# r4dl/StopThePop-Rasterization

Measured on AMD Instinct MI355X. Metric: fwd+bwd frames/sec at 1920×1080, 1M Gaussians; PSNR vs reference, higher is better.
Workload: dtype f32

## Files before the change

### stopthepop-rasterization_amd/csrc/stp_api.hip

```cpp
#include "stp_internal.h"

#include <algorithm>
#include <atomic>
#include <chrono>
#include <cstdio>
#include <cstdlib>
#include <cstring>
#include <mutex>
#include <string>
#include <unordered_map>
#include <vector>

namespace stp {

static thread_local std::string g_last_error;
static bool g_timing = false;

struct StageTimer {
    static constexpr int SETS = 64, EV = 8;
    static constexpr int HIST = 1024;
    struct Set { hipEvent_t ev[EV]; bool have[EV]; bool used; long seq; std::chrono::steady_clock::time_point host[EV]; };
    Set sets[SETS] = {};
    bool created = false;
    int cur = 0;
// ... 603 lines not shown
                const float* cam_pos, float tan_fovx, float tan_fovy, int prefiltered, float* out_color, int* radii, int debug,
                void* stream)
{
    hipStream_t st = (hipStream_t)stream;
    const ForwardSplit split = t_forward_split;
    t_forward_split = ForwardSplit{};
    struct SplitGuard {
        const ForwardSplit& s; hipStream_t st; bool done = false;
        ~SplitGuard() { if (s.armed && !done) (void)hipEventRecord(s.event, st); }
    } split_guard{split, st};
    if (!settings || !geometry_alloc || !binning_alloc || !image_alloc) return fail(STP_ERR_INVALID_ARGUMENT, "null settings or allocator");
    if (P < 0 || width <= 0 || height <= 0) return fail(STP_ERR_INVALID_ARGUMENT, "bad sizes");
    if (P == 0) return 0;
    if (!means3D || !opacities || !background || !viewmatrix || !projmatrix || !inv_viewprojmatrix || !cam_pos || !out_color)
        return fail(STP_ERR_INVALID_ARGUMENT, "null required input");
    if (int rc = check_settings(*settings, false)) return rc;
    if (!colors_precomp && !shs) return fail(STP_ERR_INVALID_ARGUMENT, "neither SHs nor precomputed colours given");
    if (!cov3D_precomp && !(scales && rotations)) return fail(STP_ERR_INVALID_ARGUMENT, "neither scale/rotation nor precomputed covariance given");
    const bool with_inv = requires_depth_along_ray(*settings);
    if (with_inv && !(scales && rotations)) return fail(STP_ERR_NEEDS_SCALE_ROTATION, "sorted modes need scales and rotations");

    FrameParams f;
    fill_frame(f, P, D, M, background, width, height, *settings, means3D, shs, colors_precomp, opacities, scales, scale_modifier,
               rotations, cov3D_precomp, viewmatrix, projmatrix, inv_viewprojmatrix, cam_pos, tan_fovx, tan_fovy, prefiltered);

    size_t geom_bytes = 0;
    carve_geometry(nullptr, (size_t)P, with_inv, &geom_bytes);
    char* geom_ptr = (char*)geometry_alloc(geometry_user, geom_bytes);
    if (!geom_ptr) return fail(STP_ERR_ALLOC, "geometry allocator returned NULL");
    GeometryState g = carve_geometry(geom_ptr, (size_t)P, with_inv, nullptr);
    if (!radii) radii = g.internal_radii;

    Mailbox mb;
    if (int rc = acquire_mailbox(&mb)) return rc;
    const uint64_t gkey = guess_key(f);
    const unsigned gidx = (unsigned)((gkey >> 1) % GUESS_SLOTS);
    SizeGuess& gslot = g_guess[mb.device][gidx];
    uint32_t* const log_need_word = g_mailboxes[mb.device].log_need + gidx;
    size_t img_bytes = 0;
    const bool with_log = uses_blend_log(*settings);
    const int log_depth = with_log ? log_depth_for(gslot, gkey) : 0;
    f.log_depth = log_depth;
    f.log_need = with_log ? log_need_word : nullptr;
    const uint32_t log_tag = (uint32_t)((gkey >> 40) & 0xFFFFu) | 1u;
    f.log_tag = log_tag;
    carve_image(nullptr, width, height, f.ty0, f.ty1, log_depth, &img_bytes);
    char* img_ptr = (char*)image_alloc(image_user, img_bytes);
    if (!img_ptr) return fail(STP_ERR_ALLOC, "image allocator returned NULL");
    ImageState img = carve_image(img_ptr, width, height, f.ty0, f.ty1, log_depth, nullptr);

    static const char* const sort_env = std::getenv("STP_SORT");
    static const bool tile_local_sort = !(sort_env && std::strcmp(sort_env, "radix") == 0);
    static const bool atomic_bin = sort_env && std::strcmp(sort_env, "counters") == 0;

    static const char* const scan_env = std::getenv("STP_SCAN");
    static const bool two_level_scan = !(scan_env && std::strcmp(scan_env, "rocprim") == 0);
    if (!two_level_scan) { g.block_sums = nullptr; g.block_prefix = nullptr; }

    g_timer.begin_forward();
    g_timer.mark(0, st);
    STP_TRY(launch_frame_init(g, img, f.gx * f.ty0, f.gx * (f.ty1 - f.ty0), with_log, atomic_bin, st), "frame init launch");
    STP_TRY(launch_preprocess(f, g, radii, atomic_bin ? img.tile_counts : nullptr, st), "preprocess launch");
    STP_DEBUG_SYNC("preprocess");
    if (!two_level_scan) STP_TRY(launch_scan(f, g, st), "inclusive scan");
    STP_DEBUG_SYNC("scan");
    if (atomic_bin) STP_TRY(launch_tile_scan(f, img, st), "tile scan");

    if (two_level_scan) STP_TRY(launch_block_prefix_mailbox(f, g, mb.dev, mb.ticket, log_need_word, st), "workgroup prefixes + mailbox launch");
    else STP_TRY(launch_mailbox(g.point_offsets + (P - 1), g.status + 1, mb.dev, mb.ticket, log_need_word, st), "mailbox launch");
    STP_TRY(hipEventRecord(mb.ev, st), "record mailbox event");
    SideStream* const side = side_stream(mb.device);
    SideJoin colours{mb.done, st, false};
    static const char* const late_env = std::getenv("STP_COLOUR_LATE");
    static const bool colour_late = !(late_env && late_env[0] == '0');
    auto colour_on_side = [&]() -> int {
        STP_TRY(hipStreamWaitEvent(side->stream, mb.ev, 0), "side stream wait");
        STP_TRY(launch_sh_color(f, g, radii, side->stream), "SH colour launch");
        if (hipError_t e = hipEventRecord(mb.done, side->stream); e != hipSuccess) {
            (void)hipStreamSynchronize(side->stream);
            return fail_hip(e, "record colour event");
        }
        colours.pending = true;
        return 0;
    };
    if (side) {
        if (!colour_late) { if (int rc = colour_on_side()) return rc; }
    } else STP_TRY(launch_sh_color(f, g, radii, st), "SH colour launch");
    static const char* const bin_env = std::getenv("STP_BINNING");
    static const bool speculative = !(bin_env && std::strcmp(bin_env, "exact") == 0);
    const int run_ahead_mode = g_run_ahead.load(std::memory_order_relaxed);
    const bool run_ahead = run_ahead_mode != 0;
    size_t bin_have = 0;
    char* bin_ptr = nullptr;
    const uint32_t guess = (speculative && gslot.key.load(std::memory_order_acquire) == gkey) ? gslot.R.load(std::memory_order_relaxed) : 0u;
    const bool ahead = run_ahead && guess > 0 && (run_ahead_mode == 1 || guess < RUN_AHEAD_AUTO_MAX) && two_level_scan && !atomic_bin && !debug;
    const uint32_t cap = guess + guess / 8 + (ahead ? 1024u : 0u);
    if (guess > 0) {
        carve_binning(nullptr, (size_t)cap, &bin_have);
        bin_ptr = (char*)binning_alloc(binning_user, bin_have);
        if (!bin_ptr) return fail(STP_ERR_ALLOC, "binning allocator returned NULL");
    }
    static const char* const mbx_env = std::getenv("STP_MAILBOX");
    static const bool mbx_spin = !(mbx_env && std::strcmp(mbx_env, "event") == 0);
    auto wait_mailbox = [&]() -> int {
        if (mbx_spin) {
            for (unsigned it = 1;; it++) {
// ... 216 lines not shown
```

### stopthepop-rasterization_amd/csrc/stp_blend.h

```cpp
#pragma once

#include "stp_device.h"

namespace stp {

struct RenderArgs {
    int W, H, gx, ty0, ty1;
    const uint2* ranges;
    const uint32_t* point_list;
    const float2* means2D;
    const float4* conic_opacity;
    const float4* cov3D_inv;
    const float* features;
    const float4* entA;
    const float4* entB;
    const float4* entC;
    const float4* entD;
    const float4* entF;
    const float* inv_vp;
    const float* cam;
    const float* bg;
    float* final_T;
    uint32_t* n_contrib;
    float* out_color;
    const float* pixel_colors;
    const float* dL_dpix;
    float* grad_rec;
    int grad_stride;
    uint32_t* blend_log;
    int log_depth;
    uint32_t* log_need;
    uint32_t log_tag;
    uint32_t* tile_flags;
    const uint32_t* tile_order;
    int flag_mode;
    int debug_depth;
    const float* means3D;
};

typedef uint16_t log_t;
constexpr int LOG_MAX_LIST = 65535;
#ifndef STP_LOG_DEPTH
#define STP_LOG_DEPTH 192
#endif
constexpr int BLEND_LOG_DEPTH = STP_LOG_DEPTH, BLEND_LOG_DEPTH_MIN = 32, BLEND_LOG_DEPTH_MAX = 512;
constexpr int LOG_BLOCK = 4;
constexpr int LOG_PIECE_SHIFT = 3;
constexpr int BLEND_LOG_SPARE = 8;
__host__ __device__ __forceinline__ size_t log_wave_bytes(int depth) { return (size_t)(depth + BLEND_LOG_SPARE) * 64 * sizeof(uint16_t); }
__device__ __forceinline__ char* log_wave_slice(uint32_t* blend_log, int tile, int wave, int depth)
{
    return reinterpret_cast<char*>(blend_log) + (size_t)(tile * 4 + wave) * log_wave_bytes(depth);
}
inline bool log_blocked(const StpSettings& s) { return s.sort_mode == 2; }
template <bool BLOCKED> __device__ __forceinline__ uint32_t log_record_offset(uint32_t j2, uint32_t lane16)
{
    if constexpr (BLOCKED) return (((j2 << 6) & ~(128u * LOG_BLOCK - 1u)) | lane16) | (j2 & (2u * LOG_BLOCK - 2u));
    else return (j2 << 6) | (lane16 >> (LOG_PIECE_SHIFT - 1));
}
struct BlockedLogCursor {
    char* wave;
    uint32_t cap2;
    uint32_t piece;
    uint32_t j2 = 0u;
    uint32_t lo = 0u, hi = 0u;
    __device__ __forceinline__ void append(bool upd, int pay)
    {
        if (upd) {
            lo = __builtin_amdgcn_alignbit(hi, lo, 16);
            hi = __builtin_amdgcn_alignbit((uint32_t)pay, hi, 16);
            if ((j2 & 6u) == 6u && j2 < cap2) *reinterpret_cast<uint2*>(wave + log_record_offset<true>(j2 & ~6u, piece)) = make_uint2(lo, hi);
        }
        j2 += upd ? 2u : 0u;
    }
    __device__ __forceinline__ int records() const { return (int)(j2 >> 1); }
    __device__ __forceinline__ void flush()
    {
        const uint32_t have = (j2 >> 1) & 3u;
        if (have != 0u && (j2 & ~6u) < cap2) {
            const unsigned long long acc = ((((unsigned long long)hi) << 32) | lo) >> (16u * (4u - have));
            *reinterpret_cast<uint2*>(wave + log_record_offset<true>(j2 & ~6u, piece)) = make_uint2((uint32_t)acc, (uint32_t)(acc >> 32));
        }
    }
};

__device__ __forceinline__ void report_log_need(uint32_t* word, int nrec, uint32_t tag)
{
    int m = nrec;
#pragma unroll
    for (int off = 32; off > 0; off >>= 1) m = max(m, __shfl_xor(m, off));
// ... 230 lines not shown
```

### stopthepop-rasterization_amd/csrc/stp_internal.h

```cpp
#pragma once

#include <hip/hip_runtime.h>
#include <cstdint>
#include <cstddef>
#include <cstdlib>
#include <string>

#include "../../include/stp_raster.h"

namespace stp {

constexpr int TILE = 16;
constexpr size_t ALIGN = 256;

enum SortMode { MODE_GLOBAL = 0, MODE_FULL = 1, MODE_KBUFFER = 2, MODE_HIER = 3 };
enum SortOrder { ORDER_Z = 0, ORDER_DISTANCE = 1, ORDER_PTD_CENTER = 2, ORDER_PTD_MAX = 3 };

inline bool uses_blend_log(const StpSettings& s)
{
    return s.record_blend_log != 0 && s.debug_visualization == 0 && (s.sort_mode == MODE_HIER || s.sort_mode == MODE_KBUFFER);
}

inline int subtile_mask_kind(const StpSettings& s)
{
// ... 61 lines not shown
    int log_depth;
};

struct BinningState {
    uint32_t* header;
    uint32_t* point_list;
    uint32_t* point_list_unsorted;
    uint64_t* keys;
    uint64_t* keys_unsorted;
    char* sort_temp;
    size_t sort_temp_bytes;
    float4* entA;
    float4* entB;
    float4* entC;
    float4* entD;
    float4* entF;
};

constexpr uint32_t STP_HEADER_MAGIC_BINNING = 0x42505453u, STP_HEADER_MAGIC_IMAGE = 0x49505453u;
struct NamedOffset { const char* name; size_t offset; size_t count; };

GeometryState carve_geometry(char* base, size_t P, bool with_inv, size_t* total, NamedOffset* names = nullptr, int* n_names = nullptr);
ImageState carve_image(char* base, int W, int H, int ty0, int ty1, int log_depth , size_t* total, NamedOffset* names = nullptr, int* n_names = nullptr);
BinningState carve_binning(char* base, size_t R, size_t* total, NamedOffset* names = nullptr, int* n_names = nullptr);

int blend_log_rows(int depth);
int blend_log_default_depth();
int blend_log_clamp_depth(int d);
size_t scan_temp_bytes(size_t P);
size_t sort_temp_bytes(size_t R);

struct FrameParams {
    int P, D, M, W, H, gx, gy;
    int ty0, ty1;
    float focal_x, focal_y, tan_fovx, tan_fovy, scale_modifier;
    StpSettings s;
    const float* background;
    const float* means3D;
    const float* shs;
    const float* colors_precomp;
    const float* opacities;
    const float* scales;
    const float* rotations;
    const float* cov3D_precomp;
    const float* viewmatrix;
    const float* projmatrix;
    const float* inv_viewprojmatrix;
    const float* cam_pos;
    int prefiltered;
    int log_depth;
    uint32_t* log_need;
    uint32_t log_tag;
    int split_launch = 0;
    int wild_cov;
};

struct BackwardParams {
    const float* pixel_colors;
    const float* dL_dpix;
    float* grad_rec;
    int grad_stride;
    int clear_rec;
    int chunk, chunks;
    float* dL_dmean2D;
    float* dL_dopacity;
    float* dL_dcolor;
    float* dL_dmean3D;
    float* dL_dcov3D;
    float* dL_dsh;
    float* dL_dscale;
    float* dL_drot;
};

hipError_t launch_preprocess(const FrameParams& f, const GeometryState& g, int* radii, uint32_t* tile_counts, hipStream_t st);
hipError_t launch_frame_init(const GeometryState& g, const ImageState& img, int tile0, int n_tiles, bool with_log, bool tile_counters, hipStream_t st);
hipError_t launch_scan(const FrameParams& f, const GeometryState& g, hipStream_t st);
bool tile_order_enabled();
inline bool tile_order_used(const FrameParams& f) { return tile_order_enabled() && f.gx * (f.ty1 - f.ty0) > 1024; }
bool gather_order_enabled();
int gather_order_mode();
hipError_t launch_tile_order(const FrameParams& f, const ImageState& img, hipStream_t st);
hipError_t launch_sh_color(const FrameParams& f, const GeometryState& g, const int* radii, hipStream_t st);
hipError_t launch_mailbox(const uint32_t* last_offset, const uint32_t* status, uint32_t* mailbox_dev, uint32_t ticket, uint32_t* log_need, hipStream_t st);
hipError_t launch_block_prefix_mailbox(const FrameParams& f, const GeometryState& g, uint32_t* mailbox_dev, uint32_t ticket, uint32_t* log_need, hipStream_t st);
hipError_t launch_duplicate(const FrameParams& f, const GeometryState& g, const int* radii, const BinningState& b, uint32_t* tile_cursor, uint32_t cap, uint32_t header_cap, uint32_t* zero_ptr, size_t zero_words, hipStream_t st);
hipError_t launch_tile_scan(const FrameParams& f, const ImageState& img, hipStream_t st);
hipError_t launch_bin_pad(const BinningState& b, const ImageState& img, int R, hipStream_t st);
hipError_t launch_sort(const FrameParams& f, const BinningState& b, int R, bool tile_bits_only, bool zeroed, hipStream_t st);
void sort_zero_region(const BinningState& b, size_t R, uint32_t tiles, uint32_t** ptr, size_t* words);
hipError_t launch_tile_sort_gather(const FrameParams& f, const GeometryState& g, const BinningState& b, const ImageState& img, int R, bool unordered, hipStream_t st);
hipError_t launch_ranges(const FrameParams& f, const BinningState& b, const ImageState& img, int R, hipStream_t st);
hipError_t launch_gather_entries(const FrameParams& f, const GeometryState& g, const BinningState& b, int R, hipStream_t st);
hipError_t launch_render_forward(const FrameParams& f, const GeometryState& g, const BinningState& b, const ImageState& img,
                                 float* out_color, hipStream_t st, std::string* err);
hipError_t launch_render_debug_finish(const FrameParams& f, const ImageState& img, float* out_color, hipStream_t st);
hipError_t launch_render_backward(const FrameParams& f, const GeometryState& g, const BinningState& b, const ImageState& img,
                                  const BackwardParams& bw, hipStream_t st, std::string* err);
hipError_t launch_preprocess_backward(const FrameParams& f, const GeometryState& g, const int* radii, const BackwardParams& bw, hipStream_t st);
hipError_t launch_mark_visible(int P, const float* means3D, const float* viewmatrix, uint8_t* present, hipStream_t st);

uint32_t higher_msb(uint32_t n);

}
```

### stopthepop-rasterization_amd/csrc/stp_render_hier.inc

```
#include "stp_internal.h"
#include "stp_blend.h"

namespace stp {

#ifdef STP_HIER_STATS
static __device__ unsigned long long g_hier_stats[16];
#if defined(STP_INST_MODE) && STP_INST_MODE == 2 && STP_INST_MID == 8
extern "C" int stp_debug_hier_stats(unsigned long long* out16)
{
    hipError_t e = hipMemcpyFromSymbol(out16, HIP_SYMBOL(g_hier_stats), sizeof(unsigned long long) * 16);
    unsigned long long z[16] = {};
    (void)hipMemcpyToSymbol(HIP_SYMBOL(g_hier_stats), z, sizeof(z));
    return (int)e;
}
#endif
#endif

namespace {

#ifndef STP_BWD_WIN
#define STP_BWD_WIN 256
#endif
#ifndef STP_BWD_RING
#define STP_BWD_RING 512
// ... 36 lines not shown
    static __host__ __device__ constexpr size_t wave_mask(int MID) { return ring_cs(MID) + (size_t)BWD_RING * 4; }
    static __host__ __device__ constexpr size_t total(int MID, int mode) { return mode == 1 ? wave_mask(MID) + 16 : hfifo(MID) + 64 * (size_t)HF_CAP * 4; }
};

__device__ __forceinline__ int hier_remap_tile(int wg, int n_wg)
{
    const int q = n_wg >> 3, r = n_wg & 7;
    const int xcd = wg & 7, k = wg >> 3;
    return (xcd < r ? xcd * (q + 1) : r * (q + 1) + (xcd - r) * q) + k;
}

constexpr int MODE_FWD = 0, MODE_BWD = 1, MODE_FWD_RECORD = 2, MODE_FWD_DEPTH = 3;

template <int HEAD, int MID, bool CULL, int MODE, bool FRCP>
__global__ void __launch_bounds__(256, MODE == MODE_BWD ? STP_BWD_WAVES : (HEAD == 4 && MID == 8 && FRCP) ? STP_FWD_WAVES : 4) render_hier_kernel(const RenderArgs a)
{
    constexpr bool FRESH_QUAD = MODE != MODE_BWD && HEAD == 4 && MID == 8 && FRCP && STP_FWD_WAVES >= 5 && CULL;
    constexpr bool BACKWARD = MODE == MODE_BWD;
    constexpr bool RECORD = MODE == MODE_FWD_RECORD;
    constexpr bool DEPTHVIZ = MODE == MODE_FWD_DEPTH;
    constexpr bool USE_POS = true;
    extern __shared__ __attribute__((aligned(16))) char smem[];
    constexpr int OLDN = (MID - 4) / 4;

    const int lane = (int)(threadIdx.x & 63);
    const int w = __builtin_amdgcn_readfirstlane((int)(threadIdx.x >> 6));
    const int s = lane >> 4;
    const int x = lane & 15;
    const int m = x >> 2;
    const int q = x & 3;

    const int rows = a.ty1 - a.ty0;
    const int t = a.tile_order ? (int)a.tile_order[blockIdx.x] : hier_remap_tile((int)blockIdx.x, a.gx * rows);
    const int tile_x = t % a.gx, tile_y = a.ty0 + t / a.gx;
    const uint2 range = a.ranges[tile_y * a.gx + tile_x];
    if constexpr (BACKWARD) {
        if (a.flag_mode == 1 && a.tile_flags[tile_y * a.gx + tile_x] == 0u) return;
    }

    const int cx = tile_x * TILE + 4 * s, cy = tile_y * TILE + 4 * w;
    const int px = cx + 2 * (m & 1) + (q & 1), py = cy + 2 * (m >> 1) + (q >> 1);
    const bool inside = px < a.W && py < a.H;
    bool active = inside;
    if constexpr (!BACKWARD) {
        if (range.y <= range.x) {
            if (inside) {
                const size_t N = (size_t)a.W * a.H, pid = (size_t)a.W * py + px;
                a.final_T[pid] = 1.0f;
                if constexpr (RECORD) a.n_contrib[pid] = 0u;
                if constexpr (DEPTHVIZ) { a.out_color[pid] = 0.0f; a.out_color[N + pid] = 1.0f; }
                else { a.out_color[pid] = a.bg[0]; a.out_color[N + pid] = a.bg[1]; a.out_color[2 * N + pid] = a.bg[2]; }
            }
            return;
        }
    }

    const int st = w * 4 + s;
    auto fresh_lane = [&]() __attribute__((always_inline)) -> int {
        int l;
        asm volatile("v_mbcnt_lo_u32_b32 %0, -1, 0\n\tv_mbcnt_hi_u32_b32 %0, -1, %0" : "=v"(l));
        return l;
    };
#define STP_ROW_VIEW(L)                                                                                                  \
    const int lrow_ = (L);                                               \
    const int x = lrow_ & 15;                                                                                            \
    const int st_r = w * 4 + (lrow_ >> 4);                                                                               \
    float* const tk = reinterpret_cast<float*>(smem + HierLds::tail_key()) + st_r * 64;                                  \
    int* const ti = reinterpret_cast<int*>(smem + HierLds::tail_id()) + st_r * 64;                                       \
    float* const nk = reinterpret_cast<float*>(smem + HierLds::new_key()) + st_r * 32;                                   \
    int* const ni = reinterpret_cast<int*>(smem + HierLds::new_id()) + st_r * 32;                                        \
    int* const fifo = reinterpret_cast<int*>(smem + HierLds::fifo(MID)) + st_r * FIFO_GROUPS * 16;
    struct QuadView { int q; float* mk; int* mi; int* hfifo; };
#define STP_QUAD_VIEW(L)                                                                                                 \
    const int lquad_ = (L);                                              \
    const int q = lquad_ & 3;                                                                                            \
    const uint32_t qi_ = (uint32_t)(w * 16) + ((uint32_t)lquad_ >> 2);                                                   \
    const uint32_t qmid_ = (MID & (MID - 1)) == 0 ? qi_ << __builtin_ctz(MID) : qi_ * (uint32_t)MID;  \
    float* const mk = reinterpret_cast<float*>(smem + HierLds::mid_key()) + qmid_;                                       \
    int* const mi = reinterpret_cast<int*>(smem + HierLds::mid_id(MID)) + qmid_;                                         \
    float* const mray = reinterpret_cast<float*>(smem + HierLds::mid_rays(MID)) + (qi_ << 2);                            \
    int* const hfifo = reinterpret_cast<int*>(smem + HierLds::hfifo(MID)) + (qi_ << __builtin_ctz(HF_CAP));             \
    const QuadView qv{q, mk, mi, hfifo}; (void)qv; (void)mray;

    const float3 cam = make_float3(a.cam[0], a.cam[1], a.cam[2]);
    const float3 pix_dir = view_ray(a.inv_vp, cam, (float)px, (float)py, a.W, a.H);
    if (q == 0) {
        float* const mray = reinterpret_cast<float*>(smem + HierLds::mid_rays(MID)) + (st * 4 + m) * 4;
        const float3 md = view_ray(a.inv_vp, cam, (float)cx + 0.5f + 2.0f * (float)(m & 1), (float)cy + 0.5f + 2.0f * (float)(m >> 1), a.W, a.H);
        mray[0] = md.x; mray[1] = md.y; mray[2] = md.z; mray[3] = 0.0f;
    }
#define STP_STAGE_VIEW(L)                                                                                                \
    const int lstage_ = (L);                                             \
    const int half = lstage_ >> 5, e = lstage_ & 31;                                                                           \
    const int sxA = tile_x * TILE + 4 * (2 * half), sxB = sxA + 4;                                                       \
    float* const tray = reinterpret_cast<float*>(smem + HierLds::rays(MID)) + (w * 2 + half) * 8;                        \
    float* const nkA = reinterpret_cast<float*>(smem + HierLds::new_key()) + (w * 4 + 2 * half) * 32;                    \
    int* const niA = reinterpret_cast<int*>(smem + HierLds::new_id()) + (w * 4 + 2 * half) * 32;
    {
    STP_STAGE_VIEW(lane)
    if (e == 0) {
        const float3 tA = view_ray(a.inv_vp, cam, (float)sxA + 1.5f, (float)cy + 1.5f, a.W, a.H);
        const float3 tB = view_ray(a.inv_vp, cam, (float)sxB + 1.5f, (float)cy + 1.5f, a.W, a.H);
        tray[0] = tA.x; tray[1] = tA.y; tray[2] = tA.z; tray[3] = 0.0f;
        tray[4] = tB.x; tray[5] = tB.y; tray[6] = tB.z; tray[7] = 0.0f;
    }
    }
// ... 739 lines not shown
```

### stopthepop-rasterization_amd/csrc/stp_render_tile.hip

```cpp
#include <cstdlib>
#include <cstring>
#include "stp_internal.h"
#include "stp_blend.h"

namespace stp {

namespace {

constexpr int BLOCK = 256;

__device__ __forceinline__ int remap_tile(int wg, int n_wg)
{
    const int q = n_wg >> 3, r = n_wg & 7;
    const int xcd = wg & 7, k = wg >> 3;
    return (xcd < r ? xcd * (q + 1) : r * (q + 1) + (xcd - r) * q) + k;
}

__device__ __forceinline__ float wave_sum(float v)
{
    int t;
    t = __builtin_amdgcn_mov_dpp(__float_as_int(v), 0xB1, 0xF, 0xF, true); v += __int_as_float(t);
    t = __builtin_amdgcn_mov_dpp(__float_as_int(v), 0x4E, 0xF, 0xF, true); v += __int_as_float(t);
    t = __builtin_amdgcn_mov_dpp(__float_as_int(v), 0x141, 0xF, 0xF, true); v += __int_as_float(t);
    t = __builtin_amdgcn_mov_dpp(__float_as_int(v), 0x140, 0xF, 0xF, true); v += __int_as_float(t);
// ... 296 lines not shown
            const float4 eCj = s_C[j];
            const float4 co = s_D[j];
            const float dx = eCj.y - pxf, dy = eCj.z - pyf;
            const float power = blend_power(dx, dy, co);
            if (power > 0.0f) continue;
            const float G = exp_blend(power);
            const float alpha = fminf(0.99f, co.w * G);
            if (alpha < ALPHA_THRESHOLD) continue;
            const float depth = depth_along_ray_ent(s_A[j], s_B[j], eCj, dir);
            if (depth < 0.0f) continue;
            win.insert(depth, BACKWARD ? __float_as_int(eCj.w) : i * BLOCK + j, BACKWARD ? G : 0.0f);
        }
    }
    if (!done)
        while (win.num > 0 && !done) blend_one();

    if constexpr (!BACKWARD) {
        if (c.inside) {
            const size_t N = (size_t)a.W * a.H, pid = (size_t)a.W * c.py + c.px;
            a.final_T[pid] = fp.T;
            a.n_contrib[pid] = RECORD ? (uint32_t)nrec : contributor;
            if constexpr (DEPTHVIZ) {
                a.out_color[pid] = depth_acc;
                a.out_color[N + pid] = fp.T;
            } else {
                a.out_color[pid] = fp.C[0] + fp.T * a.bg[0];
                a.out_color[N + pid] = fp.C[1] + fp.T * a.bg[1];
                a.out_color[2 * N + pid] = fp.C[2] + fp.T * a.bg[2];
            }
        }
        if constexpr (RECORD) {
            if (nrec > a.log_depth || total > LOG_MAX_LIST) a.tile_flags[c.tile] = 1u;
            report_log_need(a.log_need, nrec, a.log_tag);
        }
    }
}

}

static RenderArgs make_args(const FrameParams& f, const GeometryState& g, const BinningState& b, const ImageState& img)
{
    RenderArgs a{};
    a.W = f.W; a.H = f.H; a.gx = f.gx; a.ty0 = f.ty0; a.ty1 = f.ty1;
    a.ranges = img.ranges; a.point_list = b.point_list; a.means2D = g.means2D; a.conic_opacity = g.conic_opacity;
    a.cov3D_inv = g.cov3D_inv; a.features = f.colors_precomp ? f.colors_precomp : g.rgb;
    a.inv_vp = f.inv_viewprojmatrix; a.cam = f.cam_pos; a.bg = f.background;
    a.entA = b.entA; a.entB = b.entB; a.entC = b.entC; a.entD = b.entD; a.entF = b.entF;
    a.final_T = img.final_T; a.n_contrib = img.n_contrib;
    a.blend_log = img.blend_log; a.tile_flags = img.tile_flags; a.flag_mode = 0;
    static const bool counters = [] { const char* e = std::getenv("STP_SORT"); return e && std::strcmp(e, "counters") == 0; }();
    a.tile_order = (tile_order_used(f) && !counters && !f.split_launch) ? img.tile_cursor + f.gx * f.ty0 : nullptr;
    a.log_depth = img.log_depth; a.log_need = f.log_need; a.log_tag = f.log_tag;
    a.debug_depth = f.s.debug_visualization == STP_DEBUG_DEPTH ? 1 : 0; a.means3D = f.means3D;
    return a;
}

hipError_t launch_hier_fwd(const FrameParams& f, const RenderArgs& a, hipStream_t st, std::string* err);
hipError_t launch_hier_bwd(const FrameParams& f, const RenderArgs& a, hipStream_t st, std::string* err);
hipError_t launch_hier_rec(const FrameParams& f, const RenderArgs& a, hipStream_t st, std::string* err);
hipError_t launch_hier_dbg(const FrameParams& f, const RenderArgs& a, hipStream_t st, std::string* err);
hipError_t launch_depth_colormap(float* out_color, int N, uint32_t* minmax, hipStream_t st);
hipError_t launch_hier_replay(const FrameParams& f, const RenderArgs& a, hipStream_t st);
hipError_t launch_full_fwd(const FrameParams& f, const RenderArgs& a, hipStream_t st);
hipError_t launch_kbuffer_wave(int mode, const FrameParams& f, const RenderArgs& a, hipStream_t st, bool* handled);

template <int MODE> static hipError_t launch_kbuffer(const FrameParams& f, const RenderArgs& a, hipStream_t st)
{
    const dim3 grid(f.gx * (f.ty1 - f.ty0)), block(BLOCK);
    const int w = f.s.queue_per_pixel;
#define STP_KB(WIN) hipLaunchKernelGGL((render_kbuffer_kernel<WIN, MODE>), grid, block, 0, st, a)
    if (w <= 1) STP_KB(1);
    else if (w <= 2) STP_KB(2);
    else if (w <= 4) STP_KB(4);
    else if (w <= 8) STP_KB(8);
    else if (w <= 12) STP_KB(12);
    else if (w <= 16) STP_KB(16);
    else if (w <= 20) STP_KB(20);
    else STP_KB(24);
#undef STP_KB
    return hipGetLastError();
}

hipError_t launch_render_forward(const FrameParams& f, const GeometryState& g, const BinningState& b, const ImageState& img,
                                 float* out_color, hipStream_t st, std::string* err)
{
    RenderArgs a = make_args(f, g, b, img);
    a.out_color = out_color;
    const dim3 grid(f.gx * (f.ty1 - f.ty0)), block(BLOCK);
    if (grid.x == 0) return hipSuccess;
    switch (f.s.sort_mode) {
    case MODE_GLOBAL:
        hipLaunchKernelGGL(render_global_fwd_kernel, grid, block, 0, st, a);
        return hipGetLastError();
    case MODE_KBUFFER: {
        static const char* const kb_env = std::getenv("STP_KBUFFER");
        static const bool kb_tile = kb_env && std::strcmp(kb_env, "tile") == 0;
        if (!kb_tile) {
            bool handled = false;
            const hipError_t e = launch_kbuffer_wave(a.debug_depth ? KB_FWD_DEPTH : uses_blend_log(f.s) ? KB_FWD_RECORD : KB_FWD, f, a, st, &handled);
            if (handled) return e;
        }
        if (a.debug_depth) return launch_kbuffer<KB_FWD_DEPTH>(f, a, st);
        return uses_blend_log(f.s) ? launch_kbuffer<KB_FWD_RECORD>(f, a, st) : launch_kbuffer<KB_FWD>(f, a, st);
    }
    case MODE_FULL: return launch_full_fwd(f, a, st);
    case MODE_HIER:
        if (a.debug_depth) return launch_hier_dbg(f, a, st, err);
        return uses_blend_log(f.s) ? launch_hier_rec(f, a, st, err) : launch_hier_fwd(f, a, st, err);
    default: if (err) *err = "invalid sort mode"; return hipErrorInvalidValue;
    }
}

hipError_t launch_render_debug_finish(const FrameParams& f, const ImageState& img, float* out_color, hipStream_t st)
{
    if (f.s.debug_visualization != STP_DEBUG_DEPTH) return hipSuccess;
    return launch_depth_colormap(out_color, f.W * f.H, img.dbg_minmax, st);
}

hipError_t launch_render_backward(const FrameParams& f, const GeometryState& g, const BinningState& b, const ImageState& img,
                                  const BackwardParams& bw, hipStream_t st, std::string* err)
{
    RenderArgs a = make_args(f, g, b, img);
    a.pixel_colors = bw.pixel_colors; a.dL_dpix = bw.dL_dpix; a.grad_rec = bw.grad_rec; a.grad_stride = bw.grad_stride;
    const dim3 grid(f.gx * (f.ty1 - f.ty0)), block(BLOCK);
    if (grid.x == 0) return hipSuccess;
    switch (f.s.sort_mode) {
    case MODE_GLOBAL:
        hipLaunchKernelGGL(render_global_bwd_kernel, grid, block, 0, st, a);
        return hipGetLastError();
    case MODE_KBUFFER:
        if (uses_blend_log(f.s)) {
            hipError_t e = launch_hier_replay(f, a, st);
            if (e != hipSuccess) return e;
            a.flag_mode = 1;
        }
        return launch_kbuffer<KB_BWD>(f, a, st);
    case MODE_HIER:
        if (uses_blend_log(f.s)) {
            hipError_t e = launch_hier_replay(f, a, st);
            if (e != hipSuccess) return e;
            a.flag_mode = 1;
        }
        return launch_hier_bwd(f, a, st, err);
    default: if (err) *err = "Backward not supported for full per-pixel sort"; return hipErrorInvalidValue;
    }
}

}
```

### stopthepop-rasterization_amd/csrc/stp_tilesort.hip

```cpp
#include "stp_internal.h"
#include "stp_device.h"
#include <rocprim/block/block_radix_sort.hpp>

namespace stp {

namespace {

constexpr int TS_SMALL = 1024, TS_CAP = 4096;
#ifndef STP_GATHER_WAVES
#define STP_GATHER_WAVES 6
#endif

struct TileSortArgs {
    const uint2* ranges;
    uint64_t* keys;
    uint32_t* point_list;
    uint64_t* keys_scratch;
    uint32_t* list_scratch;
    const float4* gpack;
    const float* features;
    int id_passes;
    int gx;
    int tile0;
    const uint32_t* tile_order;
    int cull_mask;
    float4* entA; float4* entB; float4* entC; float4* entD; float4* entF;
};

__device__ __forceinline__ void write_entry(const TileSortArgs& a, size_t i, int id, int tile)
{
    const float4* __restrict__ gp = a.gpack + 4 * (size_t)id;
    const float4 pa = gp[0], pb = gp[1], pc = gp[2], pd = gp[3];
    const float3 col = make_float3(a.features[3 * (size_t)id], a.features[3 * (size_t)id + 1], a.features[3 * (size_t)id + 2]);
    a.entA[i] = pa;
    a.entB[i] = pb;
    a.entC[i] = make_float4(pc.x, pc.y, pc.z, __int_as_float(id));
    a.entD[i] = pd;
    float spare = 0.0f;
    if (a.cull_mask) spare = __uint_as_float(subtile_mask(a.cull_mask, pd, make_float2(pc.y, pc.z), tile % a.gx, tile / a.gx));
    a.entF[i] = make_float4(col.x, col.y, col.z, spare);
}

template <int IPT> struct TileRadix {
    using Sort = rocprim::block_radix_sort<uint32_t, 256, IPT, uint32_t>;
    template <class WriteEntry>
    static __device__ __forceinline__ void run(typename Sort::storage_type& st, uint64_t* keys, uint32_t* list, int n, int tid, WriteEntry&& write_entry_at)
    {
        const uint64_t tile_bits = keys[0] & 0xFFFFFFFF00000000ull;
        uint32_t k[IPT], v[IPT];
#pragma unroll
        for (int j = 0; j < IPT; j++) {
            const int i = tid * IPT + j;
            k[j] = i < n ? (uint32_t)keys[i] : 0xFFFFFFFFu;
            v[j] = i < n ? list[i] : 0xFFFFFFFFu;
        }
        __syncthreads();
        Sort().sort_to_striped(k, v, st, 0, 32);
#pragma unroll
        for (int j = 0; j < IPT; j++) {
            const int i = j * 256 + tid;
            if (i < n) {
                keys[i] = tile_bits | k[j];
                list[i] = v[j];
                write_entry_at(i, (int)v[j]);
            }
        }
    }
};

template <int CAP, int MIN_N>
__global__ void __launch_bounds__(256, (CAP == TS_SMALL ? STP_GATHER_WAVES : 4)) tile_sort_gather_kernel(const TileSortArgs a)
{
    using Radix8 = TileRadix<8>;
    using Radix16 = TileRadix<16>;
    constexpr size_t RADIX_BYTES = CAP == TS_CAP ? (sizeof(typename Radix16::Sort::storage_type) > sizeof(typename Radix8::Sort::storage_type) ? sizeof(typename Radix16::Sort::storage_type) : sizeof(typename Radix8::Sort::storage_type)) : 0;
    constexpr size_t RAW_BYTES = RADIX_BYTES > sizeof(uint64_t) * CAP ? RADIX_BYTES : sizeof(uint64_t) * CAP;
    __shared__ __attribute__((aligned(16))) char s_raw[RAW_BYTES];
    uint64_t* const s_key = reinterpret_cast<uint64_t*>(s_raw);
    static_assert(CAP != TS_CAP || RAW_BYTES >= sizeof(int) * 13 * 256, "the long-segment path keeps its counters in the sort's LDS area");
    const int tid = (int)threadIdx.x;
    const int n_wg = (int)gridDim.x, wg = (int)blockIdx.x;
    const int xq = n_wg >> 3, xr = n_wg & 7, xcd = wg & 7;
    const int tile = a.tile0 + (a.tile_order ? (int)a.tile_order[wg] : (xcd < xr ? xcd * (xq + 1) : xr * (xq + 1) + (xcd - xr) * xq) + (wg >> 3));
    const uint2 range = a.ranges[tile];
    const int n = (int)(range.y - range.x);
    if (n <= MIN_N || (CAP == TS_SMALL && n > TS_SMALL)) return;
    uint64_t* const keys = a.keys + range.x;
    uint32_t* const list = a.point_list + range.x;

    if constexpr (CAP == TS_CAP) {
        if (n <= CAP && a.id_passes == 0) {
            auto we = [&](int i, int id) __attribute__((always_inline)) { if (a.gpack) write_entry(a, (size_t)range.x + i, id, tile); };
            if (n <= 2048) Radix8::run(*reinterpret_cast<typename Radix8::Sort::storage_type*>(s_raw), keys, list, n, tid, we);
            else Radix16::run(*reinterpret_cast<typename Radix16::Sort::storage_type*>(s_raw), keys, list, n, tid, we);
            return;
        }
    }
    if (n <= CAP) {
        int m = 2;
        while (m < n) m <<= 1;
        const uint64_t tile_bits = keys[0] & 0xFFFFFFFF00000000ull;
        for (int i = tid; i < m; i += 256) {
            s_key[i] = i < n ? ((keys[i] << 32) | list[i]) : ~0ull;
        }
        __syncthreads();
        for (int k = 2; k <= m; k <<= 1)
            for (int j = k >> 1; j > 0; j >>= 1) {
                for (int c = tid; c < (m >> 1); c += 256) {
                    const int lo = ((c & ~(j - 1)) << 1) | (c & (j - 1));
                    const int hi = lo | j;
                    const bool up = (lo & k) == 0;
                    const uint64_t x = s_key[lo], y = s_key[hi];
                    if ((x > y) == up) { s_key[lo] = y; s_key[hi] = x; }
                }
                const int j_next = j > 1 ? (j >> 1) : k;
                const bool last = j == 1 && k == m;
                if (j > 64 || j_next > 64 || last) __syncthreads();
                else wave_sync();
            }
        for (int i = tid; i < n; i += 256) {
            const uint64_t k = s_key[i];
            const int id = (int)(uint32_t)k;
            keys[i] = tile_bits | (k >> 32);
            list[i] = (uint32_t)id;
            if (a.gpack) write_entry(a, (size_t)range.x + i, id, tile);
        }
        return;
    }

    if constexpr (CAP == TS_SMALL) return;
    int* const s_hist = reinterpret_cast<int*>(s_raw);
    int* const s_wcnt = s_hist + 256;
    int* const s_hall = s_hist + 5 * 256;
    uint64_t* src_k = keys; uint32_t* src_v = list;
    uint64_t* dst_k = a.keys_scratch + range.x; uint32_t* dst_v = a.list_scratch + range.x;
    const int n_pass = a.id_passes + 4;
    const int wv = tid >> 6, ln = tid & 63;
    const unsigned long long lt_mask = (1ull << ln) - 1ull;
    int done_passes = 0;
    for (int i = tid; i < 8 * 256; i += 256) s_hall[i] = 0;
    __syncthreads();
    {
        const int n4 = n & ~1023;
        for (int i0 = 0; i0 < n; i0 += 1024) {
            uint64_t k[4]; uint32_t v[4]; bool ok[4];
#pragma unroll
            for (int r = 0; r < 4; r++) { const int i = i0 + 256 * r + tid; ok[r] = i0 < n4 || i < n; k[r] = ok[r] ? src_k[i] : 0ull; v[r] = (ok[r] && a.id_passes) ? src_v[i] : 0u; }
#pragma unroll
            for (int r = 0; r < 4; r++)
                if (ok[r]) {
                    for (int p = 0; p < a.id_passes; p++) atomicAdd(&s_hall[256 * p + (int)((v[r] >> (8 * p)) & 0xFF)], 1);
#pragma unroll
                    for (int p = 0; p < 4; p++) atomicAdd(&s_hall[256 * (a.id_passes + p) + (int)((k[r] >> (8 * p)) & 0xFF)], 1);
                }
        }
    }
    __syncthreads();
    for (int pass = 0; pass < n_pass; pass++) {
        const bool on_id = pass < a.id_passes;
        const int shift = 8 * (on_id ? pass : pass - a.id_passes);
        auto digit = [&](uint64_t k, uint32_t v) __attribute__((always_inline)) { return (int)(((on_id ? (uint64_t)v : k) >> shift) & 0xFF); };
        s_hist[tid] = s_hall[256 * pass + tid];
#pragma unroll
        for (int r = 0; r < 4; r++) s_wcnt[256 * r + tid] = 0;
        __syncthreads();
        const bool same = s_hist[digit(src_k[0], src_v[0])] == n;
        __syncthreads();
        if (same) continue;
        if (tid < 64) {
            int c[4], sum = 0;
#pragma unroll
            for (int k = 0; k < 4; k++) { c[k] = s_hist[4 * tid + k]; sum += c[k]; }
            int inc = sum;
#pragma unroll
            for (int o = 1; o < 64; o <<= 1) { const int v = __shfl_up(inc, o); if (tid >= o) inc += v; }
            int run = inc - sum;
#pragma unroll
            for (int k = 0; k < 4; k++) { s_hist[4 * tid + k] = run; run += c[k]; }
        }
// ... 9 lines not shown
            }
#pragma unroll
            for (int r = 0; r < 4; r++) {
                d[r] = valid[r] ? digit(k[r], v[r]) : 0;
                unsigned long long peers = __ballot(valid[r]);
#pragma unroll
                for (int bit = 0; bit < 8; bit++) {
                    const bool one = ((d[r] >> bit) & 1) != 0;
                    const unsigned long long bal = __ballot(one);
                    peers &= one ? bal : ~bal;
                }
                rank[r] = __popcll(peers & lt_mask);
                if (valid[r] && rank[r] == 0) atomicAdd(&s_wcnt[256 * r + d[r]], __popcll(peers) << (8 * wv));
            }
            __syncthreads();
            auto fields = [](unsigned int wc) __attribute__((always_inline)) { return (int)((wc & 0xFFu) + ((wc >> 8) & 0xFFu) + ((wc >> 16) & 0xFFu) + (wc >> 24)); };
#pragma unroll
            for (int r = 0; r < 4; r++) {
                if (valid[r]) {
                    int below = 0;
#pragma unroll
                    for (int rr = 0; rr < 4; rr++)
                        if (rr < r) below += fields((unsigned int)s_wcnt[256 * rr + d[r]]);
                    const unsigned int wc = (unsigned int)s_wcnt[256 * r + d[r]];
                    below += (int)((wv > 0 ? (wc & 0xFFu) : 0u) + (wv > 1 ? ((wc >> 8) & 0xFFu) : 0u) + (wv > 2 ? ((wc >> 16) & 0xFFu) : 0u));
                    const int at = s_hist[d[r]] + below + rank[r];
                    dst_k[at] = k[r];
                    dst_v[at] = v[r];
                }
            }
            __syncthreads();
            {
                int tot = 0;
#pragma unroll
                for (int r = 0; r < 4; r++) {
                    const unsigned int wc = (unsigned int)s_wcnt[256 * r + tid];
                    if (wc != 0u) { tot += fields(wc); s_wcnt[256 * r + tid] = 0; }
                }
                s_hist[tid] += tot;
            }
            __syncthreads();
        }
        uint64_t* tk = src_k; src_k = dst_k; dst_k = tk;
        uint32_t* tv = src_v; src_v = dst_v; dst_v = tv;
        done_passes++;
        __threadfence_block();
        __syncthreads();
    }
    if (done_passes & 1) {
        for (int i = tid; i < n; i += 256) { keys[i] = src_k[i]; list[i] = src_v[i]; }
        __threadfence_block();
        __syncthreads();
    }
    if (a.gpack) {
#pragma unroll 4
        for (int i = tid; i < n; i += 256) write_entry(a, (size_t)range.x + i, (int)list[i], tile);
    }
}

}

hipError_t launch_tile_sort_gather(const FrameParams& f, const GeometryState& g, const BinningState& b, const ImageState& img, int R, bool unordered, hipStream_t st)
{
    if (R <= 0) return hipSuccess;
    TileSortArgs a{};
    a.id_passes = 0;
    if (unordered)
        for (unsigned int top = (unsigned int)(f.P > 1 ? f.P - 1 : 1); top; top >>= 8) a.id_passes++;
    a.ranges = img.ranges; a.keys = b.keys; a.point_list = b.point_list; a.keys_scratch = b.keys_unsorted; a.list_scratch = b.point_list_unsorted;
    const bool entries = f.s.sort_mode == MODE_HIER || f.s.sort_mode == MODE_KBUFFER;
    a.gpack = entries ? g.gpack : nullptr;
    a.features = f.colors_precomp ? f.colors_precomp : g.rgb;
    a.gx = f.gx;
    a.tile0 = f.gx * f.ty0;
    a.cull_mask = subtile_mask_kind(f.s);
    const int gmode = (tile_order_used(f) && !unordered) ? gather_order_mode() : 0;
    a.tile_order = gmode == 1 ? img.tile_counts + f.gx * f.ty0 : gmode == 2 ? img.tile_cursor + f.gx * f.ty0 : nullptr;
    a.entA = b.entA; a.entB = b.entB; a.entC = b.entC; a.entD = b.entD; a.entF = b.entF;
    const int n_tiles = f.gx * (f.ty1 - f.ty0);
    if (n_tiles <= 0) return hipSuccess;
    hipLaunchKernelGGL((tile_sort_gather_kernel<TS_SMALL, 0>), dim3(n_tiles), dim3(256), 0, st, a);
    hipLaunchKernelGGL((tile_sort_gather_kernel<TS_CAP, TS_SMALL>), dim3(n_tiles), dim3(256), 0, st, a);
    return hipGetLastError();
}

}
```

Before: 446.1.

## Fuse small-tile sort and entry gather into hierarchical forward render kernel

For hierarchical sort mode, tiles with at most TS_SMALL entries are no longer sorted and gathered by a separate kernel launch. The forward render kernel instead sorts their keys bitonically in shared memory and writes the entry arrays before blending. This removes one kernel launch and a global round trip between sort and render for small tiles. In exchange the render kernel takes on extra shared-memory pressure and synchronisation, and it re-reads the entries it just wrote through global memory. The sort code is moved into a shared header so both paths can use it.

```diff
diff --git a/stopthepop-rasterization_amd/csrc/stp_api.hip b/stopthepop-rasterization_amd/csrc/stp_api.hip
--- a/stopthepop-rasterization_amd/csrc/stp_api.hip
+++ b/stopthepop-rasterization_amd/csrc/stp_api.hip
@@ -679,6 +679,9 @@
     static const char* const sort_env = std::getenv("STP_SORT");
     static const bool tile_local_sort = !(sort_env && std::strcmp(sort_env, "radix") == 0);
     static const bool atomic_bin = sort_env && std::strcmp(sort_env, "counters") == 0;
+    static const char* const fused_env = std::getenv("STP_FUSED_GATHER");
+    static const bool fused_gather = !(fused_env && fused_env[0] == '0');
+    f.fused_gather = fused_gather && tile_local_sort && !atomic_bin && f.s.sort_mode == MODE_HIER && f.s.debug_visualization != STP_DEBUG_DEPTH ? 1 : 0;
 
     static const char* const scan_env = std::getenv("STP_SCAN");
     static const bool two_level_scan = !(scan_env && std::strcmp(scan_env, "rocprim") == 0);
diff --git a/stopthepop-rasterization_amd/csrc/stp_blend.h b/stopthepop-rasterization_amd/csrc/stp_blend.h
--- a/stopthepop-rasterization_amd/csrc/stp_blend.h
+++ b/stopthepop-rasterization_amd/csrc/stp_blend.h
@@ -1,6 +1,7 @@
 #pragma once
 
 #include "stp_device.h"
+#include "stp_tilesort.h"
 
 namespace stp {
 
@@ -36,6 +37,8 @@
     int flag_mode;
     int debug_depth;
     const float* means3D;
+    int fused_gather;
+    EntryGather gather;
 };
 
 typedef uint16_t log_t;
diff --git a/stopthepop-rasterization_amd/csrc/stp_internal.h b/stopthepop-rasterization_amd/csrc/stp_internal.h
--- a/stopthepop-rasterization_amd/csrc/stp_internal.h
+++ b/stopthepop-rasterization_amd/csrc/stp_internal.h
@@ -137,6 +137,7 @@
     uint32_t* log_need;
     uint32_t log_tag;
     int split_launch = 0;
+    int fused_gather = 0;
     int wild_cov;
 };
 
diff --git a/stopthepop-rasterization_amd/csrc/stp_render_hier.inc b/stopthepop-rasterization_amd/csrc/stp_render_hier.inc
--- a/stopthepop-rasterization_amd/csrc/stp_render_hier.inc
+++ b/stopthepop-rasterization_amd/csrc/stp_render_hier.inc
@@ -112,6 +112,14 @@
                 else { a.out_color[pid] = a.bg[0]; a.out_color[N + pid] = a.bg[1]; a.out_color[2 * N + pid] = a.bg[2]; }
             }
             return;
+        }
+    }
+    if constexpr (MODE == MODE_FWD || MODE == MODE_FWD_RECORD) {
+        const int n = (int)(range.y - range.x);
+        if (a.fused_gather && n <= TS_SMALL) {
+            tile_sort_gather_lds(a.gather, reinterpret_cast<uint64_t*>(smem), tile_y * a.gx + tile_x, range, n, (int)threadIdx.x);
+            __threadfence_block();
+            __syncthreads();
         }
     }
 
diff --git a/stopthepop-rasterization_amd/csrc/stp_render_tile.hip b/stopthepop-rasterization_amd/csrc/stp_render_tile.hip
--- a/stopthepop-rasterization_amd/csrc/stp_render_tile.hip
+++ b/stopthepop-rasterization_amd/csrc/stp_render_tile.hip
@@ -372,6 +372,10 @@
     a.tile_order = (tile_order_used(f) && !counters && !f.split_launch) ? img.tile_cursor + f.gx * f.ty0 : nullptr;
     a.log_depth = img.log_depth; a.log_need = f.log_need; a.log_tag = f.log_tag;
     a.debug_depth = f.s.debug_visualization == STP_DEBUG_DEPTH ? 1 : 0; a.means3D = f.means3D;
+    a.fused_gather = 0;
+    a.gather.keys = b.keys; a.gather.point_list = b.point_list; a.gather.gpack = g.gpack; a.gather.features = a.features;
+    a.gather.gx = f.gx; a.gather.cull_mask = subtile_mask_kind(f.s);
+    a.gather.entA = b.entA; a.gather.entB = b.entB; a.gather.entC = b.entC; a.gather.entD = b.entD; a.gather.entF = b.entF;
     return a;
 }
 
@@ -426,6 +430,7 @@
     case MODE_FULL: return launch_full_fwd(f, a, st);
     case MODE_HIER:
         if (a.debug_depth) return launch_hier_dbg(f, a, st, err);
+        a.fused_gather = f.fused_gather;
         return uses_blend_log(f.s) ? launch_hier_rec(f, a, st, err) : launch_hier_fwd(f, a, st, err);
     default: if (err) *err = "invalid sort mode"; return hipErrorInvalidValue;
     }
diff --git a/stopthepop-rasterization_amd/csrc/stp_tilesort.h b/stopthepop-rasterization_amd/csrc/stp_tilesort.h
--- /dev/null
+++ b/stopthepop-rasterization_amd/csrc/stp_tilesort.h
@@ -0,0 +1,67 @@
+#pragma once
+
+#include "stp_device.h"
+
+namespace stp {
+
+constexpr int TS_SMALL = 1024;
+
+struct EntryGather {
+    uint64_t* keys;
+    uint32_t* point_list;
+    const float4* gpack;
+    const float* features;
+    int gx;
+    int cull_mask;
+    float4* entA; float4* entB; float4* entC; float4* entD; float4* entF;
+};
+
+__device__ __forceinline__ void write_entry(const EntryGather& a, size_t i, int id, int tile)
+{
+    const float4* __restrict__ gp = a.gpack + 4 * (size_t)id;
+    const float4 pa = gp[0], pb = gp[1], pc = gp[2], pd = gp[3];
+    const float3 col = make_float3(a.features[3 * (size_t)id], a.features[3 * (size_t)id + 1], a.features[3 * (size_t)id + 2]);
+    a.entA[i] = pa;
+    a.entB[i] = pb;
+    a.entC[i] = make_float4(pc.x, pc.y, pc.z, __int_as_float(id));
+    a.entD[i] = pd;
+    float spare = 0.0f;
+    if (a.cull_mask) spare = __uint_as_float(subtile_mask(a.cull_mask, pd, make_float2(pc.y, pc.z), tile % a.gx, tile / a.gx));
+    a.entF[i] = make_float4(col.x, col.y, col.z, spare);
+}
+
+__device__ __forceinline__ void tile_sort_gather_lds(const EntryGather& a, uint64_t* s_key, int tile, uint2 range, int n, int tid)
+{
+    uint64_t* const keys = a.keys + range.x;
+    uint32_t* const list = a.point_list + range.x;
+    int m = 2;
+    while (m < n) m <<= 1;
+    const uint64_t tile_bits = keys[0] & 0xFFFFFFFF00000000ull;
+    for (int i = tid; i < m; i += 256) {
+        s_key[i] = i < n ? ((keys[i] << 32) | list[i]) : ~0ull;
+    }
+    __syncthreads();
+    for (int k = 2; k <= m; k <<= 1)
+        for (int j = k >> 1; j > 0; j >>= 1) {
+            for (int c = tid; c < (m >> 1); c += 256) {
+                const int lo = ((c & ~(j - 1)) << 1) | (c & (j - 1));
+                const int hi = lo | j;
+                const bool up = (lo & k) == 0;
+                const uint64_t x = s_key[lo], y = s_key[hi];
+                if ((x > y) == up) { s_key[lo] = y; s_key[hi] = x; }
+            }
+            const int j_next = j > 1 ? (j >> 1) : k;
+            const bool last = j == 1 && k == m;
+            if (j > 64 || j_next > 64 || last) __syncthreads();
+            else wave_sync();
+        }
+    for (int i = tid; i < n; i += 256) {
+        const uint64_t k = s_key[i];
+        const int id = (int)(uint32_t)k;
+        keys[i] = tile_bits | (k >> 32);
+        list[i] = (uint32_t)id;
+        if (a.gpack) write_entry(a, (size_t)range.x + i, id, tile);
+    }
+}
+
+}
diff --git a/stopthepop-rasterization_amd/csrc/stp_tilesort.hip b/stopthepop-rasterization_amd/csrc/stp_tilesort.hip
--- a/stopthepop-rasterization_amd/csrc/stp_tilesort.hip
+++ b/stopthepop-rasterization_amd/csrc/stp_tilesort.hip
@@ -1,45 +1,26 @@
 #include "stp_internal.h"
 #include "stp_device.h"
+#include "stp_tilesort.h"
 #include <rocprim/block/block_radix_sort.hpp>
 
 namespace stp {
 
 namespace {
 
-constexpr int TS_SMALL = 1024, TS_CAP = 4096;
+constexpr int TS_CAP = 4096;
 #ifndef STP_GATHER_WAVES
 #define STP_GATHER_WAVES 6
 #endif
 
 struct TileSortArgs {
     const uint2* ranges;
-    uint64_t* keys;
-    uint32_t* point_list;
     uint64_t* keys_scratch;
     uint32_t* list_scratch;
-    const float4* gpack;
-    const float* features;
     int id_passes;
-    int gx;
     int tile0;
     const uint32_t* tile_order;
-    int cull_mask;
-    float4* entA; float4* entB; float4* entC; float4* entD; float4* entF;
+    EntryGather e;
 };
-
-__device__ __forceinline__ void write_entry(const TileSortArgs& a, size_t i, int id, int tile)
-{
-    const float4* __restrict__ gp = a.gpack + 4 * (size_t)id;
-    const float4 pa = gp[0], pb = gp[1], pc = gp[2], pd = gp[3];
-    const float3 col = make_float3(a.features[3 * (size_t)id], a.features[3 * (size_t)id + 1], a.features[3 * (size_t)id + 2]);
-    a.entA[i] = pa;
-    a.entB[i] = pb;
-    a.entC[i] = make_float4(pc.x, pc.y, pc.z, __int_as_float(id));
-    a.entD[i] = pd;
-    float spare = 0.0f;
-    if (a.cull_mask) spare = __uint_as_float(subtile_mask(a.cull_mask, pd, make_float2(pc.y, pc.z), tile % a.gx, tile / a.gx));
-    a.entF[i] = make_float4(col.x, col.y, col.z, spare);
-}
 
 template <int IPT> struct TileRadix {
     using Sort = rocprim::block_radix_sort<uint32_t, 256, IPT, uint32_t>;
@@ -85,46 +66,19 @@
     const uint2 range = a.ranges[tile];
     const int n = (int)(range.y - range.x);
     if (n <= MIN_N || (CAP == TS_SMALL && n > TS_SMALL)) return;
-    uint64_t* const keys = a.keys + range.x;
-    uint32_t* const list = a.point_list + range.x;
+    uint64_t* const keys = a.e.keys + range.x;
+    uint32_t* const list = a.e.point_list + range.x;
 
     if constexpr (CAP == TS_CAP) {
         if (n <= CAP && a.id_passes == 0) {
-            auto we = [&](int i, int id) __attribute__((always_inline)) { if (a.gpack) write_entry(a, (size_t)range.x + i, id, tile); };
+            auto we = [&](int i, int id) __attribute__((always_inline)) { if (a.e.gpack) write_entry(a.e, (size_t)range.x + i, id, tile); };
             if (n <= 2048) Radix8::run(*reinterpret_cast<typename Radix8::Sort::storage_type*>(s_raw), keys, list, n, tid, we);
             else Radix16::run(*reinterpret_cast<typename Radix16::Sort::storage_type*>(s_raw), keys, list, n, tid, we);
             return;
         }
     }
     if (n <= CAP) {
-        int m = 2;
-        while (m < n) m <<= 1;
-        const uint64_t tile_bits = keys[0] & 0xFFFFFFFF00000000ull;
-        for (int i = tid; i < m; i += 256) {
-            s_key[i] = i < n ? ((keys[i] << 32) | list[i]) : ~0ull;
-        }
-        __syncthreads();
-        for (int k = 2; k <= m; k <<= 1)
-            for (int j = k >> 1; j > 0; j >>= 1) {
-                for (int c = tid; c < (m >> 1); c += 256) {
-                    const int lo = ((c & ~(j - 1)) << 1) | (c & (j - 1));
-                    const int hi = lo | j;
-                    const bool up = (lo & k) == 0;
-                    const uint64_t x = s_key[lo], y = s_key[hi];
-                    if ((x > y) == up) { s_key[lo] = y; s_key[hi] = x; }
-                }
-                const int j_next = j > 1 ? (j >> 1) : k;
-                const bool last = j == 1 && k == m;
-                if (j > 64 || j_next > 64 || last) __syncthreads();
-                else wave_sync();
-            }
-        for (int i = tid; i < n; i += 256) {
-            const uint64_t k = s_key[i];
-            const int id = (int)(uint32_t)k;
-            keys[i] = tile_bits | (k >> 32);
-            list[i] = (uint32_t)id;
-            if (a.gpack) write_entry(a, (size_t)range.x + i, id, tile);
-        }
+        tile_sort_gather_lds(a.e, s_key, tile, range, n, tid);
         return;
     }
 
@@ -240,9 +194,9 @@
         __threadfence_block();
         __syncthreads();
     }
-    if (a.gpack) {
+    if (a.e.gpack) {
 #pragma unroll 4
-        for (int i = tid; i < n; i += 256) write_entry(a, (size_t)range.x + i, (int)list[i], tile);
+        for (int i = tid; i < n; i += 256) write_entry(a.e, (size_t)range.x + i, (int)list[i], tile);
     }
 }
 
@@ -255,19 +209,19 @@
     a.id_passes = 0;
     if (unordered)
         for (unsigned int top = (unsigned int)(f.P > 1 ? f.P - 1 : 1); top; top >>= 8) a.id_passes++;
-    a.ranges = img.ranges; a.keys = b.keys; a.point_list = b.point_list; a.keys_scratch = b.keys_unsorted; a.list_scratch = b.point_list_unsorted;
+    a.ranges = img.ranges; a.e.keys = b.keys; a.e.point_list = b.point_list; a.keys_scratch = b.keys_unsorted; a.list_scratch = b.point_list_unsorted;
     const bool entries = f.s.sort_mode == MODE_HIER || f.s.sort_mode == MODE_KBUFFER;
-    a.gpack = entries ? g.gpack : nullptr;
-    a.features = f.colors_precomp ? f.colors_precomp : g.rgb;
-    a.gx = f.gx;
+    a.e.gpack = entries ? g.gpack : nullptr;
+    a.e.features = f.colors_precomp ? f.colors_precomp : g.rgb;
+    a.e.gx = f.gx;
     a.tile0 = f.gx * f.ty0;
-    a.cull_mask = subtile_mask_kind(f.s);
+    a.e.cull_mask = subtile_mask_kind(f.s);
     const int gmode = (tile_order_used(f) && !unordered) ? gather_order_mode() : 0;
     a.tile_order = gmode == 1 ? img.tile_counts + f.gx * f.ty0 : gmode == 2 ? img.tile_cursor + f.gx * f.ty0 : nullptr;
-    a.entA = b.entA; a.entB = b.entB; a.entC = b.entC; a.entD = b.entD; a.entF = b.entF;
+    a.e.entA = b.entA; a.e.entB = b.entB; a.e.entC = b.entC; a.e.entD = b.entD; a.e.entF = b.entF;
     const int n_tiles = f.gx * (f.ty1 - f.ty0);
     if (n_tiles <= 0) return hipSuccess;
-    hipLaunchKernelGGL((tile_sort_gather_kernel<TS_SMALL, 0>), dim3(n_tiles), dim3(256), 0, st, a);
+    if (!f.fused_gather) hipLaunchKernelGGL((tile_sort_gather_kernel<TS_SMALL, 0>), dim3(n_tiles), dim3(256), 0, st, a);
     hipLaunchKernelGGL((tile_sort_gather_kernel<TS_CAP, TS_SMALL>), dim3(n_tiles), dim3(256), 0, st, a);
     return hipGetLastError();
 }
```

After: 455.2 (median of 6 runs). 2.0% higher.
